# brownvc/matryodshka

Hardware: AMD Instinct MI355X
Metric: novel-view frames/sec, 640x320 ODS->32-sphere MSI infer+render (higher is better)
Workload: dtype f32

## Files before the change

matryodshka_amd/csrc/cnn_x3.hip:

```cpp
#include "cnn_device.h"

namespace {

#ifndef MSI_X3_EARLY_DMA
#define MSI_X3_EARLY_DMA 0
#endif
#ifndef MSI_X3_NSTG
#define MSI_X3_NSTG 0
#endif
#ifndef MSI_X2_NSTG
#define MSI_X2_NSTG 3
#endif
constexpr int x3_rate_y(int RATE) { return RATE == 3 ? 1 : RATE; }
constexpr int x3_rate_x(int RATE) { return RATE == 3 ? 2 : RATE; }
constexpr int x3_nstg(int RATE, int NPL) { return NPL == 2 ? MSI_X2_NSTG : (MSI_X3_NSTG ? MSI_X3_NSTG : (RATE == 2 ? 3 : 2)); }
template <int RATE, int NS = x3_nstg(RATE, 3), int NPL = 3, int TH = 4>
struct HaloGeomX3 {
  static constexpr int PW = 16 + 2 * x3_rate_x(RATE), PH = TH + 2 * x3_rate_y(RATE), NPX = PW * PH;
  static constexpr int PIX_BYTES = NPL * 64 + 16;
  static constexpr int ROW_PITCH = ((PW * PIX_BYTES + 127) / 256) * 256 + 128;
  static constexpr int A_BYTES = PH * ROW_PITCH;
  static constexpr int B_ROW = 64;
  static constexpr int B_PLANE = 64 * B_ROW, B_STAGE = NPL * B_PLANE;
  static constexpr int NSTG = NS;
// ... 42 lines not shown
    asm("v_cvt_pk_bf16_f32 %0, %1, %2" : "=v"(h1) : "v"(y.z), "v"(y.w));
    v4f r = y - v4f{__builtin_bit_cast(float, h0 << 16), __builtin_bit_cast(float, h0 & 0xffff0000u),
                    __builtin_bit_cast(float, h1 << 16), __builtin_bit_cast(float, h1 & 0xffff0000u)};
    asm("v_cvt_pk_bf16_f32 %0, %1, %2" : "=v"(m0) : "v"(r.x), "v"(r.y));
    asm("v_cvt_pk_bf16_f32 %0, %1, %2" : "=v"(m1) : "v"(r.z), "v"(r.w));
    r = r - v4f{__builtin_bit_cast(float, m0 << 16), __builtin_bit_cast(float, m0 & 0xffff0000u),
                __builtin_bit_cast(float, m1 << 16), __builtin_bit_cast(float, m1 & 0xffff0000u)};
    asm("v_cvt_pk_bf16_f32 %0, %1, %2" : "=v"(l0) : "v"(r.x), "v"(r.y));
    asm("v_cvt_pk_bf16_f32 %0, %1, %2" : "=v"(l1) : "v"(r.z), "v"(r.w));
    if (off != 0xffffffffu) {
      *reinterpret_cast<u2x_t *>(smem + off) = u2x_t{h0, h1};
      *reinterpret_cast<u2x_t *>(smem + off + 64) = u2x_t{m0, m1};
      *reinterpret_cast<u2x_t *>(smem + off + 128) = u2x_t{l0, l1};
    }
  }
}
template <int NP>
__device__ __forceinline__ void split_mfma(f32x16 &acc, f32x16 &lo, const v4f &ah, const v4f &am, const v4f &al, const v4f &bh, const v4f &bm, const v4f &bl) {
  typedef __bf16 bf16x8 __attribute__((ext_vector_type(8)));
  typedef _Float16 f16x8 __attribute__((ext_vector_type(8)));
  if (NP == 2) {
    lo = __builtin_amdgcn_mfma_f32_32x32x16_f16(__builtin_bit_cast(f16x8, bm), __builtin_bit_cast(f16x8, ah), lo, 0, 0, 0);
    acc = __builtin_amdgcn_mfma_f32_32x32x16_f16(__builtin_bit_cast(f16x8, bh), __builtin_bit_cast(f16x8, ah), acc, 0, 0, 0);
    lo = __builtin_amdgcn_mfma_f32_32x32x16_f16(__builtin_bit_cast(f16x8, bh), __builtin_bit_cast(f16x8, am), lo, 0, 0, 0);
  } else if (NP == 6) {
    acc = __builtin_amdgcn_mfma_f32_32x32x16_bf16(__builtin_bit_cast(bf16x8, bm), __builtin_bit_cast(bf16x8, am), acc, 0, 0, 0);
    acc = __builtin_amdgcn_mfma_f32_32x32x16_bf16(__builtin_bit_cast(bf16x8, bh), __builtin_bit_cast(bf16x8, al), acc, 0, 0, 0);
    acc = __builtin_amdgcn_mfma_f32_32x32x16_bf16(__builtin_bit_cast(bf16x8, bl), __builtin_bit_cast(bf16x8, ah), acc, 0, 0, 0);
    acc = __builtin_amdgcn_mfma_f32_32x32x16_bf16(__builtin_bit_cast(bf16x8, bh), __builtin_bit_cast(bf16x8, am), acc, 0, 0, 0);
    acc = __builtin_amdgcn_mfma_f32_32x32x16_bf16(__builtin_bit_cast(bf16x8, bm), __builtin_bit_cast(bf16x8, ah), acc, 0, 0, 0);
// ... 97 lines not shown
    }
  };
  auto patch_store = [&]() __attribute__((always_inline)) {
    v4f s4 = {1.f, 1.f, 1.f, 1.f}, t4 = {0.f, 0.f, 0.f, 0.f};
    if (APPLY) ln_scale_shift(ln, g4, be4, s4, t4);
#pragma unroll
    for (int k_ = 0; k_ < NLOAD; ++k_) {
      v4f y = araw[k_];
      if (APPLY) {
        y = __builtin_elementwise_max(__builtin_elementwise_fma(y, s4, t4), v4f{0.f, 0.f, 0.f, 0.f});
        if (has_pad && !pok[k_]) y = v4f{0.f, 0.f, 0.f, 0.f};
      }
      split_store<NPL>(smem, lds_a[k_], y, amax_);
    }
  };
  const int frow = lane & 31, fh = lane >> 5, fswz = (frow >> 1) & 7;
  const unsigned lds_base = (unsigned)(size_t)(lds_void *)smem;
  const unsigned a_base = lds_base + (unsigned)((2 * MT * wm + (frow >> 4)) * G::ROW_PITCH + ((frow & 15) ^ ((frow >> 4) << 3)) * G::PIX_BYTES + fh * 16);
  unsigned b_s[2];
  (void)fswz;
#pragma unroll
  for (int s_ = 0; s_ < 2; ++s_)
    b_s[s_] = lds_base + G::A_BYTES + (wn * 32 + frow) * G::B_ROW + (((2 * s_ + fh) ^ ((frow >> 2) & 3)) << 4);
  typedef _Float16 f16x8 __attribute__((ext_vector_type(8)));
  f32x16 acc[MT][1], acc_lo, acc_lo1;
#pragma unroll
  for (int i = 0; i < MT; ++i)
#pragma unroll
    for (int r = 0; r < 16; ++r) acc[i][0][r] = acc_lo[r] = acc_lo1[r] = 0.f;

// ... 58 lines not shown
    } else {
#pragma unroll
      for (int s_ = 0; s_ < 2; ++s_) {
      ah_[s_] = s_ == 0 ? lds_read128<AOFF_>(a_base) : lds_read128<AOFF_ + 32>(a_base);
      bh_[s_] = lds_read128<0>(b_s[s_] + bst_);
      am_[s_] = s_ == 0 ? lds_read128<AOFF_ + 64>(a_base) : lds_read128<AOFF_ + 96>(a_base);
      bm_[s_] = lds_read128<G::B_PLANE>(b_s[s_] + bst_);
      al_[s_] = s_ == 0 ? lds_read128<AOFF_ + 128>(a_base) : lds_read128<AOFF_ + 160>(a_base);
      bl_[s_] = lds_read128<2 * G::B_PLANE>(b_s[s_] + bst_);
    }
#pragma unroll
      for (int s_ = 0; s_ < 2; ++s_) {
      if (s_ == 0) wait_lgkm6<6>(ah_[0], bh_[0], am_[0], bm_[0], al_[0], bl_[0]);
      else wait_lgkm6<0>(ah_[1], bh_[1], am_[1], bm_[1], al_[1], bl_[1]);
      split_mfma<3>(acc[0][0], acc_lo, ah_[s_], am_[s_], al_[s_], bh_[s_], bm_[s_], bl_[s_]);
      __builtin_amdgcn_sched_barrier(0);
      if (s_ == 0) {
        if (TAP == 0 && c + 1 < c1) patch_load(c + 1);
        if (!MSI_X3_EARLY_DMA && G::NSTG == 3) {
        if (TAP + 2 < 9) { b_issue(c, TAP + 2, (TAP + 2) % 3); }
        else if (c + 1 < c1) { b_issue(c + 1, TAP - 7, (TAP + 2) % 3); }
        }
      }
    }
    }
    {
      const bool issued_ = (TAP + 2 < 9) || (c + 1 < c1);
      if (G::NSTG == 2) {
        if (TAP == 0 && c + 1 < c1) wait_vmcnt<NLOAD + (APPLY ? 2 : 0)>();
        else wait_vmcnt<0>();
// ... 9 lines not shown
    double *s_stat = reinterpret_cast<double *>(smem);
    ln_mean_inv_pre(shard, p.ln_inv_n, p.ln_scl_src, p.status, s_stat, tid);
    ln = ln_affine_read(s_stat);
  }
  wait_vmcnt<0>();
  patch_store();
  asm volatile("s_waitcnt lgkmcnt(0)" ::: "memory");
  __builtin_amdgcn_s_barrier();
#ifdef MSI_CONV_TIMING
  const unsigned long long ts1 = __builtin_amdgcn_s_memtime();
#endif
  for (; c < c1; ++c) {
    cpar = (c - c0) & 1;
    htap(IC<0>{}); htap(IC<1>{}); htap(IC<2>{}); htap(IC<3>{}); htap(IC<4>{}); htap(IC<5>{}); htap(IC<6>{}); htap(IC<7>{}); htap(IC<8>{});
    if (c + 1 < c1) {
      patch_store();
      asm volatile("s_waitcnt lgkmcnt(0)" ::: "memory");
      __builtin_amdgcn_s_barrier();
    }
  }
  if (MSI_X2_LATE_CB && NPL == 2) load_coord_bias(p, tile_m, tile_n, tid, cbv);
  split_finish<NPL>(acc[0][0], acc_lo, amax_, lane, p.status);
  if constexpr (MT == 2 && NPL == 3) split_finish<3>(acc[1][0], acc_lo1, amax_, lane, p.status);

#ifdef MSI_CONV_TIMING
  const unsigned long long ts2 = __builtin_amdgcn_s_memtime();
  auto stamp = [&]() __attribute__((always_inline)) {
    if (p.dbg && tid == 0) {
      unsigned long long *o = p.dbg + (size_t)blockIdx.x * 24;
      o[0] = ts0; o[1] = ts1; o[2] = ts2; o[3] = __builtin_amdgcn_s_memtime(); o[22] = ts0r; o[23] = __builtin_amdgcn_s_memrealtime();
      o[4] = __builtin_amdgcn_s_getreg(4 | (31 << 11));
// ... 61 lines not shown
  static constexpr int B_ROW = 64, B_PLANE = 64 * B_ROW, B_STAGE = NP * B_PLANE;
  static constexpr int NSTG = NP == 3 ? MSI_S2X3_NSTG : 3;
  static constexpr int LDS_BYTES = A_BYTES + NSTG * B_STAGE;
  static constexpr int NLOAD = (NPX * 8 + 255) / 256;
};

#ifndef MSI_S2X_WAVES
#define MSI_S2X_WAVES 3
#endif
template <int APPLY, int NP, int TH>
__device__ __forceinline__ void conv_halo_s2_x3_body(const ConvParams &p, char *smem) {
  typedef HaloGeomS2X3<NP, TH> G;
  constexpr int PW = G::PW, NPX = G::NPX, NLOAD = G::NLOAD;
  constexpr int MT = TH / 4, NT = 1, BM = 16 * TH;
  static_assert(TH == 4 || (TH == 8 && NP == 3 && G::NSTG == 2), "the 8-row tile: six-product form, two-stage ring");
  const int tid = threadIdx.x, lane = tid & 63;
  const int wave = __builtin_amdgcn_readfirstlane(tid >> 6);
  const int wm = wave >> 1, wn = wave & 1;
  const int CH = p.cpt0;
  const TileWork w = tile_work(p, CH);
  const int c0 = w.k0, c1 = w.k1;
  const TileIndex ti = tile_index(p, w.t);
  const int tile_m = ti.tile_m, tile_n = ti.tile_n, b = ti.b;
  const int tyi = (int)udiv_magic((unsigned)tile_m, (unsigned)p.halo_tx, p.mg_htx);
  const int oh0 = tyi * TH, ow0 = (tile_m - tyi * p.halo_tx) * 16;
  const int H = p.Hin, W = p.Win, C = p.C0;
  const int S = p.ksteps;
  const int plane_bytes = p.npad * G::B_ROW;
  const __amdgpu_buffer_rsrc_t rsrc_b = __builtin_amdgcn_make_buffer_rsrc((void *)p.wpk_x3, 0, (int)((size_t)S * NP * plane_bytes), 0x00020000);
  const unsigned b_voff = (unsigned)((tile_n * 64 + wave * 16 + (lane >> 2)) * G::B_ROW + (lane & 3) * 16);
// ... 61 lines not shown
    }
  };
  auto patch_store = [&](auto U_c) __attribute__((always_inline)) {
    constexpr int U = decltype(U_c)::value;
    if (APPLY && U == 0) ln_scale_shift(LnAffine{inv_f, mu_hi, mu_lo}, g4, be4, s4, t4);
#pragma unroll
    for (int k_ = 0; k_ < NLOAD; ++k_) {
      v4f y = araw[k_];
      if (APPLY) {
        y = __builtin_elementwise_max(__builtin_elementwise_fma(y, s4, t4), v4f{0.f, 0.f, 0.f, 0.f});
        if (has_pad && !pok[U][k_]) y = v4f{0.f, 0.f, 0.f, 0.f};
      }
      split_store<NP>(smem, lds_a[k_], y, amax_);
    }
  };

  const int frow = lane & 31, fh = lane >> 5, fswz = (frow >> 1) & 7;
  const unsigned lds_base = (unsigned)(size_t)(lds_void *)smem;
  const unsigned a_base = lds_base + (unsigned)((2 * MT * wm + (frow >> 4)) * G::ROW_PITCH + ((frow & 15) ^ ((frow >> 4) << 3)) * G::PIX_BYTES + fh * 16);
  unsigned b_s[2];
  (void)fswz;
#pragma unroll
  for (int s_ = 0; s_ < 2; ++s_)
    b_s[s_] = lds_base + G::A_BYTES + (wn * 32 + frow) * G::B_ROW + (((2 * s_ + fh) ^ ((frow >> 2) & 3)) << 4);
  typedef __bf16 bf16x8 __attribute__((ext_vector_type(8), unused));
  f32x16 acc[MT][1], acc_lo, acc_lo1;
#pragma unroll
  for (int r = 0; r < 16; ++r) {
    acc_lo[r] = acc_lo1[r] = 0.f;
#pragma unroll
// ... 12 lines not shown
    if (G::NSTG == 2) {
      const int stn_ = ((J ^ cpar) & 1) ^ 1;
      if (J + 1 < 9) b_issue(c, s2_tap((J + 1) % 9), stn_);
      else if (c + 1 < c1) b_issue(c + 1, s2_tap(0), stn_);
    }
    v4f ah_[2], am_[2], al_[2], bh_[2], bm_[2], bl_[2];
    if constexpr (MT == 2) {
      constexpr int A1_ = AOFF_ + 2 * G::ROW_PITCH;
      v4f xh_[2][2], xm_[2][2], xl_[2][2];
      bh_[0] = lds_read128<0>(b_s[0] + bst_); bm_[0] = lds_read128<G::B_PLANE>(b_s[0] + bst_); bl_[0] = lds_read128<2 * G::B_PLANE>(b_s[0] + bst_);
      xh_[0][0] = lds_read128<AOFF_>(a_base); xm_[0][0] = lds_read128<AOFF_ + 64>(a_base); xl_[0][0] = lds_read128<AOFF_ + 128>(a_base);
      xh_[0][1] = lds_read128<A1_>(a_base); xm_[0][1] = lds_read128<A1_ + 64>(a_base); xl_[0][1] = lds_read128<A1_ + 128>(a_base);
      bh_[1] = lds_read128<0>(b_s[1] + bst_); bm_[1] = lds_read128<G::B_PLANE>(b_s[1] + bst_); bl_[1] = lds_read128<2 * G::B_PLANE>(b_s[1] + bst_);
      wait_lgkm6<6>(bh_[0], bm_[0], bl_[0], xh_[0][0], xm_[0][0], xl_[0][0]);
      split_mfma<3>(acc[0][0], acc_lo, xh_[0][0], xm_[0][0], xl_[0][0], bh_[0], bm_[0], bl_[0]);
      __builtin_amdgcn_sched_barrier(0);
      xh_[1][0] = lds_read128<AOFF_ + 32>(a_base); xm_[1][0] = lds_read128<AOFF_ + 96>(a_base); xl_[1][0] = lds_read128<AOFF_ + 160>(a_base);
      xh_[1][1] = lds_read128<A1_ + 32>(a_base); xm_[1][1] = lds_read128<A1_ + 96>(a_base); xl_[1][1] = lds_read128<A1_ + 160>(a_base);
      if (FIRST_ && more_) {
        if (U_ < 3) patch_load(c, IC<(U_ + 1) & 3>{});
        else patch_load(c + 1, IC<0>{});
      }
      wait_lgkm6<9>(xh_[0][1], xm_[0][1], xl_[0][1], bh_[0], bm_[0], bl_[0]);
      split_mfma<3>(acc[1][0], acc_lo1, xh_[0][1], xm_[0][1], xl_[0][1], bh_[0], bm_[0], bl_[0]);
      __builtin_amdgcn_sched_barrier(0);
      wait_lgkm6<3>(bh_[1], bm_[1], bl_[1], xh_[1][0], xm_[1][0], xl_[1][0]);
      split_mfma<3>(acc[0][0], acc_lo, xh_[1][0], xm_[1][0], xl_[1][0], bh_[1], bm_[1], bl_[1]);
      __builtin_amdgcn_sched_barrier(0);
      wait_lgkm6<0>(xh_[1][1], xm_[1][1], xl_[1][1], bh_[1], bm_[1], bl_[1]);
      split_mfma<3>(acc[1][0], acc_lo1, xh_[1][1], xm_[1][1], xl_[1][1], bh_[1], bm_[1], bl_[1]);
      __builtin_amdgcn_sched_barrier(0);
    } else {
#pragma unroll
    for (int s_ = 0; s_ < 2; ++s_) {
      ah_[s_] = s_ == 0 ? lds_read128<AOFF_>(a_base) : lds_read128<AOFF_ + 32>(a_base);
      bh_[s_] = lds_read128<0>(b_s[s_] + bst_);
      am_[s_] = s_ == 0 ? lds_read128<AOFF_ + 64>(a_base) : lds_read128<AOFF_ + 96>(a_base);
      bm_[s_] = lds_read128<G::B_PLANE>(b_s[s_] + bst_);
      if (NP == 3) {
        al_[s_] = s_ == 0 ? lds_read128<AOFF_ + 128>(a_base) : lds_read128<AOFF_ + 160>(a_base);
        bl_[s_] = lds_read128<2 * G::B_PLANE>(b_s[s_] + bst_);
      } else { al_[s_] = ah_[s_]; bl_[s_] = bh_[s_]; }
    }
#pragma unroll
    for (int s_ = 0; s_ < 2; ++s_) {
      if (NP == 3) {
        if (s_ == 0) wait_lgkm6<6>(ah_[0], bh_[0], am_[0], bm_[0], al_[0], bl_[0]);
        else wait_lgkm6<0>(ah_[1], bh_[1], am_[1], bm_[1], al_[1], bl_[1]);
      } else {
        if (s_ == 0) wait_lgkm4<4>(ah_[0], bh_[0], am_[0], bm_[0]);
        else wait_lgkm4<0>(ah_[1], bh_[1], am_[1], bm_[1]);
      }
      split_mfma<NP>(acc[0][0], acc_lo, ah_[s_], am_[s_], al_[s_], bh_[s_], bm_[s_], bl_[s_]);
      __builtin_amdgcn_sched_barrier(0);
      if (s_ == 0) {
        if (FIRST_ && more_) {
          if (U_ < 3) patch_load(c, IC<(U_ + 1) & 3>{});
          else patch_load(c + 1, IC<0>{});
        }
        if (G::NSTG == 3) {
        if (J + 2 < 9) b_issue(c, s2_tap((J + 2) % 9), (J + 2) % 3);
        else if (c + 1 < c1) b_issue(c + 1, s2_tap((J + 2) % 9), (J + 2) % 3);
        }
      }
    }
    }
    {
      const bool issued_ = (J + 2 < 9) || (c + 1 < c1);
      if (G::NSTG == 2) {
        if (FIRST_ && !LAST_ && more_) wait_vmcnt<NLOAD>();
        else wait_vmcnt<0>();
      } else if (FIRST_ && !LAST_ && more_) wait_vmcnt<NP + NLOAD>();
      else if (issued_) wait_vmcnt<NP>();
      else wait_vmcnt<0>();
    }
    __builtin_amdgcn_s_barrier();
    if (LAST_ && more_) {
      patch_store(IC<(U_ + 1) & 3>{});
      asm volatile("s_waitcnt lgkmcnt(0)" ::: "memory");
      __builtin_amdgcn_s_barrier();
    }
  };

  if (APPLY) {
    double *s_stat = reinterpret_cast<double *>(smem);
    ln_mean_inv(p.ln_sums + (size_t)b * LN_SHARDS * LN_WORDS, p.ln_inv_n, p.ln_scl_src, p.status, s_stat, tid);
    const LnAffine a = ln_affine_read(s_stat);
    inv_f = a.inv; mu_hi = a.mu_hi; mu_lo = a.mu_lo;
  }
  wait_vmcnt<0>();
  patch_store(IC<0>{});
  asm volatile("s_waitcnt lgkmcnt(0)" ::: "memory");
  __builtin_amdgcn_s_barrier();
  for (; c < c1; ++c) {
    cpar = (c - c0) & 1;
    s2step(IC<0>{}); s2step(IC<1>{}); s2step(IC<2>{}); s2step(IC<3>{}); s2step(IC<4>{});
    s2step(IC<5>{}); s2step(IC<6>{}); s2step(IC<7>{}); s2step(IC<8>{});
  }
  split_finish<NP>(acc[0][0], acc_lo, amax_, lane, p.status);
  if constexpr (MT == 2 && NP == 3) split_finish<3>(acc[1][0], acc_lo1, amax_, lane, p.status);

  if (!w.full) {
    if (!splitk_arrive<MT, NT>(p, acc, w, smem, tid)) return;
    splitk_sum<MT, NT>(p, acc, w, tid);
  }
  emit_tile<BM, 64, MODE_CONV>(p, acc, tile_m, tile_n, 0, b, tid, smem);
}

template <int APPLY, int NP>
__global__ void __launch_bounds__(256) __attribute__((amdgpu_waves_per_eu(NP == 2 ? MSI_S2X_WAVES : (MSI_S2X3_NSTG == 2 ? 3 : 2))))
conv_halo_s2_x3_kernel(const ConvParams p) {
#if defined(__HIP_DEVICE_COMPILE__)
  extern __shared__ __attribute__((aligned(16))) char smem[];
  conv_halo_s2_x3_body<APPLY, NP, 4>(p, smem);
#endif
}

template <int APPLY>
__global__ void __launch_bounds__(256) __attribute__((amdgpu_waves_per_eu(2)))
conv_halo8_s2_x3_kernel(const ConvParams p) {
#if defined(__HIP_DEVICE_COMPILE__)
// ... 11 lines not shown
  static constexpr int NLOAD = (NPX * 8 + 255) / 256;
};
#ifndef MSI_CT_MAXW
#define MSI_CT_MAXW 8
#endif
#ifndef MSI_CT3_NSTG
#define MSI_CT3_NSTG 2
#endif
template <int NP, int TH>
__device__ __forceinline__ void convt_halo_x3_body(const ConvParams &p, char *smem) {
  typedef HaloGeomCT3<(NP == 3 ? MSI_CT3_NSTG : 3), NP, TH> G;
  constexpr int PW = G::PW, NPX = G::NPX, NLOAD = G::NLOAD, NSTG = G::NSTG, PD = NSTG - 1;
  constexpr int MT = TH / 4, BM = 16 * TH;
  static_assert(NSTG == 3 || NSTG == 2, "prefetch distance two or one");
  static_assert(TH == 4 || (TH == 8 && NP == 3 && NSTG == 2), "the 8-row tile: six-product form, two-stage ring");
  const int tid = threadIdx.x, lane = tid & 63;
  const int wave = __builtin_amdgcn_readfirstlane(tid >> 6);
  const int wm = wave >> 1, wn = wave & 1;
  const int CH = p.cpt0 + p.cpt1;
  const TileWork w = tile_work(p, CH);
  const int c0 = w.k0, c1 = w.k1;
  const TileIndex ti = tile_index<TILE_ROW_PARITY>(p, w.t);
  const int ph = ti.cls, tile_m = ti.tile_m, tile_n = ti.tile_n, b = ti.b;
  const int tyi = (int)udiv_magic((unsigned)tile_m, (unsigned)p.halo_tx, p.mg_htx);
  const int oh0 = tyi * TH, ow0 = (tile_m - tyi * p.halo_tx) * 16;
  const int H = p.Hin, W = p.Win;
  const int rowup = (ph && !p.wrap) ? 0 : 1;

  const int S = p.ksteps;
  const int plane_bytes = p.npad * G::B_ROW;
// ... 74 lines not shown
      const float ih_ = src_ld ? inv_f[1] : inv_f[0], mh_ = src_ld ? mu_hi[1] : mu_hi[0], ml_ = src_ld ? mu_lo[1] : mu_lo[0];
      s4 = ih_ * g4;
      const v4f nh = {-mh_, -mh_, -mh_, -mh_}, nl = {-ml_, -ml_, -ml_, -ml_};
      t4 = __builtin_elementwise_fma(nl, s4, __builtin_elementwise_fma(nh, s4, be4));
    }
#pragma unroll
    for (int k_ = 0; k_ < NLOAD; ++k_) {
      v4f y = araw[k_];
      if (ap_) {
        y = __builtin_elementwise_max(__builtin_elementwise_fma(y, s4, t4), v4f{0.f, 0.f, 0.f, 0.f});
        if (has_pad && !pok[k_]) y = v4f{0.f, 0.f, 0.f, 0.f};
      }
      split_store<NP>(smem, lds_a[k_], y, amax_);
    }
  };

  const int frow = lane & 31, fh = lane >> 5, fswz = (frow >> 1) & 7;
  const unsigned lds_base = (unsigned)(size_t)(lds_void *)smem;
  const unsigned a_base0 = lds_base + (unsigned)((rowup + 2 * MT * wm + (frow >> 4)) * G::ROW_PITCH + ((frow & 15) ^ ((frow >> 4) << 3)) * G::PIX_BYTES + fh * 16);
  const unsigned a_base1 = rowup ? a_base0 - G::ROW_PITCH : a_base0 + G::ROW_PITCH;
  const unsigned wadj = p.wrap ? 2u * G::PIX_BYTES : 0u;
  unsigned b_s[2];
  (void)fswz;
#pragma unroll
  for (int s_ = 0; s_ < 2; ++s_)
    b_s[s_] = lds_base + G::A_BYTES + (wn * 32 + frow) * G::B_ROW + (((2 * s_ + fh) ^ ((frow >> 2) & 3)) << 4);
  typedef __bf16 bf16x8 __attribute__((ext_vector_type(8), unused));
  f32x16 acc[2][MT][1], acc_lo[2];
#pragma unroll
  for (int cl = 0; cl < 2; ++cl)
#pragma unroll
    for (int r = 0; r < 16; ++r) {
      acc_lo[cl][r] = 0.f;
#pragma unroll
      for (int i = 0; i < MT; ++i) acc[cl][i][0][r] = 0.f;
    }

  int c = c0, st = 0;
  constexpr int NPLD = NLOAD + 2;
  auto ctstep = [&](auto J_c) __attribute__((always_inline)) {
    constexpr int J = decltype(J_c)::value;
    constexpr int PWC_ = J >> 2, TH_ = (J >> 1) & 1, TW_ = J & 1;
    constexpr int COFF_ = (1 + (PWC_ ? TW_ : -TW_)) * G::PIX_BYTES;
    const unsigned ab_ = (TH_ ? a_base1 : a_base0) - ((PWC_ && TW_) ? wadj : 0u);
    v4f ah_[2], am_[2], al_[2], bh_[2], bm_[2], bl_[2];
    const unsigned bst_ = (unsigned)st * G::B_STAGE;
    bool issued_ = false;
    if (NSTG == 2) {
      constexpr int JN_ = (J + 1) & 7;
      if (J + 1 < 8) { issued_ = true; b_issue(2 * ph + (JN_ >> 2), JN_ & 3, c, st ^ 1); }
      else if (c + 1 < c1) { issued_ = true; b_issue(2 * ph + (JN_ >> 2), JN_ & 3, c + 1, st ^ 1); }
    }
    if constexpr (MT == 2) {
      constexpr int C1_ = COFF_ + 2 * G::ROW_PITCH;
      v4f xh_[2][2], xm_[2][2], xl_[2][2];
      bh_[0] = lds_read128<0>(b_s[0] + bst_); bm_[0] = lds_read128<G::B_PLANE>(b_s[0] + bst_); bl_[0] = lds_read128<2 * G::B_PLANE>(b_s[0] + bst_);
      xh_[0][0] = lds_read128<COFF_>(ab_); xm_[0][0] = lds_read128<COFF_ + 64>(ab_); xl_[0][0] = lds_read128<COFF_ + 128>(ab_);
      xh_[0][1] = lds_read128<C1_>(ab_); xm_[0][1] = lds_read128<C1_ + 64>(ab_); xl_[0][1] = lds_read128<C1_ + 128>(ab_);
      bh_[1] = lds_read128<0>(b_s[1] + bst_); bm_[1] = lds_read128<G::B_PLANE>(b_s[1] + bst_); bl_[1] = lds_read128<2 * G::B_PLANE>(b_s[1] + bst_);
      wait_lgkm6<6>(bh_[0], bm_[0], bl_[0], xh_[0][0], xm_[0][0], xl_[0][0]);
      split_mfma<6>(acc[PWC_][0][0], acc_lo[PWC_], xh_[0][0], xm_[0][0], xl_[0][0], bh_[0], bm_[0], bl_[0]);
      __builtin_amdgcn_sched_barrier(0);
      xh_[1][0] = lds_read128<COFF_ + 32>(ab_); xm_[1][0] = lds_read128<COFF_ + 96>(ab_); xl_[1][0] = lds_read128<COFF_ + 160>(ab_);
      xh_[1][1] = lds_read128<C1_ + 32>(ab_); xm_[1][1] = lds_read128<C1_ + 96>(ab_); xl_[1][1] = lds_read128<C1_ + 160>(ab_);
      if (J == 0 && c + 1 < c1) patch_load(c + 1);
      wait_lgkm6<9>(xh_[0][1], xm_[0][1], xl_[0][1], bh_[0], bm_[0], bl_[0]);
      split_mfma<6>(acc[PWC_][1][0], acc_lo[PWC_], xh_[0][1], xm_[0][1], xl_[0][1], bh_[0], bm_[0], bl_[0]);
      __builtin_amdgcn_sched_barrier(0);
      wait_lgkm6<3>(bh_[1], bm_[1], bl_[1], xh_[1][0], xm_[1][0], xl_[1][0]);
      split_mfma<6>(acc[PWC_][0][0], acc_lo[PWC_], xh_[1][0], xm_[1][0], xl_[1][0], bh_[1], bm_[1], bl_[1]);
      __builtin_amdgcn_sched_barrier(0);
      wait_lgkm6<0>(xh_[1][1], xm_[1][1], xl_[1][1], bh_[1], bm_[1], bl_[1]);
      split_mfma<6>(acc[PWC_][1][0], acc_lo[PWC_], xh_[1][1], xm_[1][1], xl_[1][1], bh_[1], bm_[1], bl_[1]);
      __builtin_amdgcn_sched_barrier(0);
    } else {
#pragma unroll
    for (int s_ = 0; s_ < 2; ++s_) {
      ah_[s_] = s_ == 0 ? lds_read128<COFF_>(ab_) : lds_read128<COFF_ + 32>(ab_);
      bh_[s_] = lds_read128<0>(b_s[s_] + bst_);
      am_[s_] = s_ == 0 ? lds_read128<COFF_ + 64>(ab_) : lds_read128<COFF_ + 96>(ab_);
      bm_[s_] = lds_read128<G::B_PLANE>(b_s[s_] + bst_);
      if (NP == 3) {
        al_[s_] = s_ == 0 ? lds_read128<COFF_ + 128>(ab_) : lds_read128<COFF_ + 160>(ab_);
        bl_[s_] = lds_read128<2 * G::B_PLANE>(b_s[s_] + bst_);
      } else { al_[s_] = ah_[s_]; bl_[s_] = bh_[s_]; }
    }
#pragma unroll
    for (int s_ = 0; s_ < 2; ++s_) {
      if (NP == 3) {
        if (s_ == 0) wait_lgkm6<6>(ah_[0], bh_[0], am_[0], bm_[0], al_[0], bl_[0]);
        else wait_lgkm6<0>(ah_[1], bh_[1], am_[1], bm_[1], al_[1], bl_[1]);
      } else {
        if (s_ == 0) wait_lgkm4<4>(ah_[0], bh_[0], am_[0], bm_[0]);
        else wait_lgkm4<0>(ah_[1], bh_[1], am_[1], bm_[1]);
      }
      split_mfma<NP>(acc[PWC_][0][0], acc_lo[PWC_], ah_[s_], am_[s_], al_[s_], bh_[s_], bm_[s_], bl_[s_]);
      __builtin_amdgcn_sched_barrier(0);
      if (s_ == 0) {
        if (J == 0 && c + 1 < c1) patch_load(c + 1);
        if (NSTG == 3) {
        int sn_ = st + PD; sn_ = sn_ >= NSTG ? sn_ - NSTG : sn_;
        constexpr int JN_ = (J + PD) & 7;
        if (J + PD < 8) { issued_ = true; b_issue(2 * ph + (JN_ >> 2), JN_ & 3, c, sn_); }
        else if (c + 1 < c1) { issued_ = true; b_issue(2 * ph + (JN_ >> 2), JN_ & 3, c + 1, sn_); }
        }
      }
    }
    }
    if (NSTG == 2) {
      if (J == 0 && c + 1 < c1) wait_vmcnt<NPLD>();
      else wait_vmcnt<0>();
// ... 10 lines not shown
    if (p.halo_apply & 1) {
      ln_mean_inv(p.ln_sums + (size_t)b * LN_SHARDS * LN_WORDS, p.ln_inv_n, p.ln_scl_src, p.status, s_stat, tid);
      const LnAffine a = ln_affine_read(s_stat);
      inv_f[0] = a.inv; mu_hi[0] = a.mu_hi; mu_lo[0] = a.mu_lo;
    }
    if (p.halo_apply & 2) {
      ln_mean_inv(p.ln_sums1 + (size_t)b * LN_SHARDS * LN_WORDS, p.ln_inv_n1, p.ln_scl_src1, p.status, s_stat, tid);
      const LnAffine a = ln_affine_read(s_stat);
      inv_f[1] = a.inv; mu_hi[1] = a.mu_hi; mu_lo[1] = a.mu_lo;
    }
  }
  wait_vmcnt<0>();
  patch_store();
  asm volatile("s_waitcnt lgkmcnt(0)" ::: "memory");
  __builtin_amdgcn_s_barrier();
  for (; c < c1; ++c) {
    ctstep(IC<0>{}); ctstep(IC<1>{}); ctstep(IC<2>{}); ctstep(IC<3>{}); ctstep(IC<4>{}); ctstep(IC<5>{}); ctstep(IC<6>{}); ctstep(IC<7>{});
    if (c + 1 < c1) {
      patch_store();
      asm volatile("s_waitcnt lgkmcnt(0)" ::: "memory");
      __builtin_amdgcn_s_barrier();
    }
  }
  if constexpr (MT == 1) {
    split_finish<NP>(acc[0][0][0], acc_lo[0], amax_, lane, p.status);
    split_finish<NP>(acc[1][0][0], acc_lo[1], amax_, lane, p.status);
  }

  if (!w.full) {
    constexpr int SLAB = BM * 64 * 4;
    if (p.tile_cnt == nullptr) {
#pragma unroll
      for (int cl = 0; cl < 2; ++cl) {
        const __amdgpu_buffer_rsrc_t rsrc_p = __builtin_amdgcn_make_buffer_rsrc((void *)(p.partial + ((size_t)w.slot * 2 + cl) * (BM * 64)), 0, SLAB, 0x00020000);
        dump_acc<MT, 1, 0>(acc[cl], rsrc_p, tid);
      }
      return;
    }
#pragma unroll
    for (int cl = 0; cl < 2; ++cl) {
      const __amdgpu_buffer_rsrc_t rsrc_p = __builtin_amdgcn_make_buffer_rsrc((void *)(p.partial + ((size_t)w.slot * 2 + cl) * (BM * 64)), 0, SLAB, 0x00020000);
      dump_acc<MT, 1, MSI_HANDOFF_AUX>(acc[cl], rsrc_p, tid);
    }
    const int nsp = w.t < p.n_main ? p.split0 : p.split;
    asm volatile("s_waitcnt vmcnt(0)" ::: "memory");
    handoff_release();
    __syncthreads();
    int *s_old = reinterpret_cast<int *>(smem);
    if (tid == 0)
      *s_old = __hip_atomic_fetch_add(p.tile_cnt + (w.t - (p.split0 == 1 ? p.n_main : 0)), 1, __ATOMIC_RELAXED, __HIP_MEMORY_SCOPE_AGENT);
    __syncthreads();
    if (*s_old != nsp - 1) return;
    handoff_acquire();
#pragma unroll
    for (int cl = 0; cl < 2; ++cl) {
      const __amdgpu_buffer_rsrc_t rsrc_t = __builtin_amdgcn_make_buffer_rsrc((void *)(p.partial + ((size_t)(w.slot - w.ks) * 2 + cl) * (BM * 64)), 0, nsp * 2 * SLAB, 0x00020000);
      sum_slabs<MT, 1, MSI_HANDOFF_AUX>(acc[cl], rsrc_t, nsp, 2 * SLAB, tid);
    }
  }
#pragma unroll
  for (int cl = 0; cl < 2; ++cl) emit_tile<BM, 64, MODE_CONVT>(p, acc[cl], tile_m, tile_n, 2 * ph + cl, b, tid);
}

template <int NP>
__global__ void __launch_bounds__(256) __attribute__((amdgpu_waves_per_eu(NP == 3 ? 3 : 2, MSI_CT_MAXW)))
convt_halo_x3_kernel(const ConvParams p) {
#if defined(__HIP_DEVICE_COMPILE__)
  extern __shared__ __attribute__((aligned(16))) char smem[];
  convt_halo_x3_body<NP, 4>(p, smem);
#endif
}

__global__ void __launch_bounds__(256) __attribute__((amdgpu_waves_per_eu(2)))
convt_halo8_x3_kernel(const ConvParams p) {
#if defined(__HIP_DEVICE_COMPILE__)
  extern __shared__ __attribute__((aligned(16))) char smem[];
// ... 49 lines not shown
```

Before: 542.5.

## Interleave next-patch bf16 split with MFMA k-steps instead of at barrier

Moves the LayerNorm-affine, ReLU and three-plane bf16 split of the prefetched next input patch out of the serial store phase at each channel boundary. The work is spread into slots behind MFMA groups across the tap/k-step loop, using sched_group_barrier hints to interleave VALU with MFMA. The split planes are kept in registers and only written to LDS at the boundary. This adds register pressure (the extra plane arrays) and can perturb the schedule. The diff also adds optional timing instrumentation behind a macro.

```diff
diff --git a/matryodshka_amd/csrc/cnn_x3.hip b/matryodshka_amd/csrc/cnn_x3.hip
--- a/matryodshka_amd/csrc/cnn_x3.hip
+++ b/matryodshka_amd/csrc/cnn_x3.hip
@@ -2,6 +2,9 @@
 
 namespace {
 
+#ifndef MSI_EARLY_SPLIT
+#define MSI_EARLY_SPLIT 28
+#endif
 #ifndef MSI_X3_EARLY_DMA
 #define MSI_X3_EARLY_DMA 0
 #endif
@@ -80,6 +83,56 @@
       *reinterpret_cast<u2x_t *>(smem + off + 128) = u2x_t{l0, l1};
     }
   }
+}
+template <int NP>
+__device__ __forceinline__ void split_planes(v4f y, unsigned &amax, unsigned (&q)[2 * NP]) {
+  if constexpr (NP == 2) {
+    typedef _Float16 h2_t __attribute__((ext_vector_type(2)));
+    f16_range_track(amax, y);
+    const h2_t ha = {(_Float16)y.x, (_Float16)y.y}, hb = {(_Float16)y.z, (_Float16)y.w};
+    const h2_t ma = {(_Float16)((y.x - (float)ha.x) * 2048.f), (_Float16)((y.y - (float)ha.y) * 2048.f)};
+    const h2_t mb = {(_Float16)((y.z - (float)hb.x) * 2048.f), (_Float16)((y.w - (float)hb.y) * 2048.f)};
+    q[0] = __builtin_bit_cast(unsigned, ha); q[1] = __builtin_bit_cast(unsigned, hb);
+    q[2] = __builtin_bit_cast(unsigned, ma); q[3] = __builtin_bit_cast(unsigned, mb);
+  } else {
+    unsigned h0, h1, m0, m1, l0, l1;
+    asm("v_cvt_pk_bf16_f32 %0, %1, %2" : "=v"(h0) : "v"(y.x), "v"(y.y));
+    asm("v_cvt_pk_bf16_f32 %0, %1, %2" : "=v"(h1) : "v"(y.z), "v"(y.w));
+    v4f r = y - v4f{__builtin_bit_cast(float, h0 << 16), __builtin_bit_cast(float, h0 & 0xffff0000u),
+                    __builtin_bit_cast(float, h1 << 16), __builtin_bit_cast(float, h1 & 0xffff0000u)};
+    asm("v_cvt_pk_bf16_f32 %0, %1, %2" : "=v"(m0) : "v"(r.x), "v"(r.y));
+    asm("v_cvt_pk_bf16_f32 %0, %1, %2" : "=v"(m1) : "v"(r.z), "v"(r.w));
+    r = r - v4f{__builtin_bit_cast(float, m0 << 16), __builtin_bit_cast(float, m0 & 0xffff0000u),
+                __builtin_bit_cast(float, m1 << 16), __builtin_bit_cast(float, m1 & 0xffff0000u)};
+    asm("v_cvt_pk_bf16_f32 %0, %1, %2" : "=v"(l0) : "v"(r.x), "v"(r.y));
+    asm("v_cvt_pk_bf16_f32 %0, %1, %2" : "=v"(l1) : "v"(r.z), "v"(r.w));
+    q[0] = h0; q[1] = h1; q[2] = m0; q[3] = m1; q[4] = l0; q[5] = l1;
+  }
+}
+template <int NP>
+__device__ __forceinline__ void planes_store(char *smem, unsigned off, const unsigned (&q)[2 * NP]) {
+  typedef unsigned u2x_t __attribute__((ext_vector_type(2)));
+  if (off != 0xffffffffu) {
+    *reinterpret_cast<u2x_t *>(smem + off) = u2x_t{q[0], q[1]};
+    *reinterpret_cast<u2x_t *>(smem + off + 64) = u2x_t{q[2], q[3]};
+    if constexpr (NP == 3) *reinterpret_cast<u2x_t *>(smem + off + 128) = u2x_t{q[4], q[5]};
+  }
+}
+__device__ __forceinline__ void planes_keep(v4f &a, unsigned (&l)[2], const unsigned (&q)[6]) {
+  a = __builtin_bit_cast(v4f, u32x4_t{q[0], q[1], q[2], q[3]});
+  l[0] = q[4]; l[1] = q[5];
+}
+__device__ __forceinline__ void mfma_valu_interleave() {
+#pragma unroll
+  for (int i = 0; i < 6; ++i) {
+    __builtin_amdgcn_sched_group_barrier(0x008, 1, 0);
+    __builtin_amdgcn_sched_group_barrier(0x002, 7, 0);
+  }
+}
+__device__ __forceinline__ void planes_kept_store(char *smem, unsigned off, const v4f &a, const unsigned (&l)[2]) {
+  const u32x4_t hm = __builtin_bit_cast(u32x4_t, a);
+  const unsigned q[6] = {hm.x, hm.y, hm.z, hm.w, l[0], l[1]};
+  planes_store<3>(smem, off, q);
 }
 template <int NP>
 __device__ __forceinline__ void split_mfma(f32x16 &acc, f32x16 &lo, const v4f &ah, const v4f &am, const v4f &al, const v4f &bh, const v4f &bm, const v4f &bl) {
@@ -207,6 +260,35 @@
       split_store<NPL>(smem, lds_a[k_], y, amax_);
     }
   };
+  constexpr bool EARLY = TH == 4 && NPL == 3 && RATE != 2 && ((MSI_EARLY_SPLIT >> 4) & 1);
+  unsigned apl[EARLY ? NLOAD : 1][2];
+  auto early_slot = [&](auto TAP_c, auto Q_c) __attribute__((always_inline)) {
+    constexpr int k_ = decltype(Q_c)::value == 1 ? decltype(TAP_c)::value - (9 - NLOAD) : -1;
+    static_assert(NLOAD <= 7, "a slot per float4 of the patch, none before tap 2");
+    if constexpr (EARLY && k_ >= 0 && k_ < NLOAD) {
+      if (APPLY && k_ == 0) {
+        v4f s4 = {1.f, 1.f, 1.f, 1.f}, t4 = {0.f, 0.f, 0.f, 0.f};
+        ln_scale_shift(ln, g4, be4, s4, t4);
+        g4 = s4; be4 = t4;
+      }
+      v4f y = araw[k_];
+      if (APPLY) {
+        y = __builtin_elementwise_max(__builtin_elementwise_fma(y, g4, be4), v4f{0.f, 0.f, 0.f, 0.f});
+        const bool zero_ = has_pad && !pok[k_];
+        y.x = zero_ ? 0.f : y.x; y.y = zero_ ? 0.f : y.y; y.z = zero_ ? 0.f : y.z; y.w = zero_ ? 0.f : y.w;
+      }
+      unsigned q_[6];
+      split_planes<3>(y, amax_, q_);
+      planes_keep(araw[k_], apl[k_], q_);
+      mfma_valu_interleave();
+    }
+  };
+  auto early_store = [&]() __attribute__((always_inline)) {
+    if constexpr (EARLY) {
+#pragma unroll
+      for (int k_ = 0; k_ < NLOAD; ++k_) planes_kept_store(smem, lds_a[k_], araw[k_], apl[k_]);
+    }
+  };
   const int frow = lane & 31, fh = lane >> 5, fswz = (frow >> 1) & 7;
   const unsigned lds_base = (unsigned)(size_t)(lds_void *)smem;
   const unsigned a_base = lds_base + (unsigned)((2 * MT * wm + (frow >> 4)) * G::ROW_PITCH + ((frow & 15) ^ ((frow >> 4) << 3)) * G::PIX_BYTES + fh * 16);
@@ -295,6 +377,7 @@
       if (s_ == 0) wait_lgkm6<6>(ah_[0], bh_[0], am_[0], bm_[0], al_[0], bl_[0]);
       else wait_lgkm6<0>(ah_[1], bh_[1], am_[1], bm_[1], al_[1], bl_[1]);
       split_mfma<3>(acc[0][0], acc_lo, ah_[s_], am_[s_], al_[s_], bh_[s_], bm_[s_], bl_[s_]);
+      if (s_ == 0) early_slot(TAP_c, IC<0>{}); else early_slot(TAP_c, IC<1>{});
       __builtin_amdgcn_sched_barrier(0);
       if (s_ == 0) {
         if (TAP == 0 && c + 1 < c1) patch_load(c + 1);
@@ -334,7 +417,8 @@
     cpar = (c - c0) & 1;
     htap(IC<0>{}); htap(IC<1>{}); htap(IC<2>{}); htap(IC<3>{}); htap(IC<4>{}); htap(IC<5>{}); htap(IC<6>{}); htap(IC<7>{}); htap(IC<8>{});
     if (c + 1 < c1) {
-      patch_store();
+      if constexpr (EARLY) early_store();
+      else patch_store();
       asm volatile("s_waitcnt lgkmcnt(0)" ::: "memory");
       __builtin_amdgcn_s_barrier();
     }
@@ -426,6 +510,9 @@
   constexpr int PW = G::PW, NPX = G::NPX, NLOAD = G::NLOAD;
   constexpr int MT = TH / 4, NT = 1, BM = 16 * TH;
   static_assert(TH == 4 || (TH == 8 && NP == 3 && G::NSTG == 2), "the 8-row tile: six-product form, two-stage ring");
+#ifdef MSI_CONV_TIMING
+  const unsigned long long ts0 = __builtin_amdgcn_s_memtime(), ts0r = __builtin_amdgcn_s_memrealtime();
+#endif
   const int tid = threadIdx.x, lane = tid & 63;
   const int wave = __builtin_amdgcn_readfirstlane(tid >> 6);
   const int wm = wave >> 1, wn = wave & 1;
@@ -517,6 +604,42 @@
       split_store<NP>(smem, lds_a[k_], y, amax_);
     }
   };
+  constexpr bool EARLY = NP == 3 && ((MSI_EARLY_SPLIT >> (TH == 8 ? 3 : 2)) & 1);
+  unsigned apl[EARLY ? NLOAD : 1][2];
+  auto early_split = [&](auto U_c, auto K_c) __attribute__((always_inline)) {
+    constexpr int U = decltype(U_c)::value, k_ = decltype(K_c)::value;
+    if constexpr (EARLY && k_ >= 0 && k_ < NLOAD) {
+      v4f y = araw[k_];
+      if (APPLY) {
+        y = __builtin_elementwise_max(__builtin_elementwise_fma(y, s4, t4), v4f{0.f, 0.f, 0.f, 0.f});
+        const bool zero_ = has_pad && !pok[U][k_];
+        y.x = zero_ ? 0.f : y.x; y.y = zero_ ? 0.f : y.y; y.z = zero_ ? 0.f : y.z; y.w = zero_ ? 0.f : y.w;
+      }
+      unsigned q_[6];
+      split_planes<3>(y, amax_, q_);
+      planes_keep(araw[k_], apl[k_], q_);
+    }
+  };
+  auto early_slot = [&](auto J_c, auto Q_c) __attribute__((always_inline)) {
+    constexpr int J = decltype(J_c)::value, U_ = s2_unit(J), NG_ = 2 * MT, Q_ = decltype(Q_c)::value;
+    constexpr int E_ = U_ == 0 ? 2 : (U_ == 3 ? 0 : 1), LASTJ_ = U_ == 0 ? 3 : (U_ == 1 ? 5 : (U_ == 2 ? 7 : 8));
+    constexpr int NS_ = E_ * NG_, SLOT_ = Q_ < 0 ? -1 : (J - (LASTJ_ - E_ + 1)) * NG_ + Q_;
+    constexpr int SPS_ = NS_ ? (NLOAD + NS_ - 1) / NS_ : 0, K0_ = NLOAD - (NS_ - SLOT_) * SPS_;
+    static_assert(SPS_ <= 3, "at most three float4s behind one MFMA group");
+    if constexpr (EARLY && E_ > 0 && SLOT_ >= 0) {
+      if constexpr (SLOT_ == 0 && E_ == 1) wait_vmcnt<NP>();
+      early_split(IC<(U_ + 1) & 3>{}, IC<K0_>{});
+      if constexpr (SPS_ >= 2) early_split(IC<(U_ + 1) & 3>{}, IC<K0_ + 1>{});
+      if constexpr (SPS_ == 3) early_split(IC<(U_ + 1) & 3>{}, IC<K0_ + 2>{});
+      if constexpr (K0_ + SPS_ > 0) mfma_valu_interleave();
+    }
+  };
+  auto early_store = [&]() __attribute__((always_inline)) {
+    if constexpr (EARLY) {
+#pragma unroll
+      for (int k_ = 0; k_ < NLOAD; ++k_) planes_kept_store(smem, lds_a[k_], araw[k_], apl[k_]);
+    }
+  };
 
   const int frow = lane & 31, fh = lane >> 5, fswz = (frow >> 1) & 7;
   const unsigned lds_base = (unsigned)(size_t)(lds_void *)smem;
@@ -559,6 +682,7 @@
       bh_[1] = lds_read128<0>(b_s[1] + bst_); bm_[1] = lds_read128<G::B_PLANE>(b_s[1] + bst_); bl_[1] = lds_read128<2 * G::B_PLANE>(b_s[1] + bst_);
       wait_lgkm6<6>(bh_[0], bm_[0], bl_[0], xh_[0][0], xm_[0][0], xl_[0][0]);
       split_mfma<3>(acc[0][0], acc_lo, xh_[0][0], xm_[0][0], xl_[0][0], bh_[0], bm_[0], bl_[0]);
+      early_slot(J_c, IC<0>{});
       __builtin_amdgcn_sched_barrier(0);
       xh_[1][0] = lds_read128<AOFF_ + 32>(a_base); xm_[1][0] = lds_read128<AOFF_ + 96>(a_base); xl_[1][0] = lds_read128<AOFF_ + 160>(a_base);
       xh_[1][1] = lds_read128<A1_ + 32>(a_base); xm_[1][1] = lds_read128<A1_ + 96>(a_base); xl_[1][1] = lds_read128<A1_ + 160>(a_base);
@@ -568,12 +692,15 @@
       }
       wait_lgkm6<9>(xh_[0][1], xm_[0][1], xl_[0][1], bh_[0], bm_[0], bl_[0]);
       split_mfma<3>(acc[1][0], acc_lo1, xh_[0][1], xm_[0][1], xl_[0][1], bh_[0], bm_[0], bl_[0]);
+      early_slot(J_c, IC<1>{});
       __builtin_amdgcn_sched_barrier(0);
       wait_lgkm6<3>(bh_[1], bm_[1], bl_[1], xh_[1][0], xm_[1][0], xl_[1][0]);
       split_mfma<3>(acc[0][0], acc_lo, xh_[1][0], xm_[1][0], xl_[1][0], bh_[1], bm_[1], bl_[1]);
+      early_slot(J_c, IC<2>{});
       __builtin_amdgcn_sched_barrier(0);
       wait_lgkm6<0>(xh_[1][1], xm_[1][1], xl_[1][1], bh_[1], bm_[1], bl_[1]);
       split_mfma<3>(acc[1][0], acc_lo1, xh_[1][1], xm_[1][1], xl_[1][1], bh_[1], bm_[1], bl_[1]);
+      early_slot(J_c, IC<3>{});
       __builtin_amdgcn_sched_barrier(0);
     } else {
 #pragma unroll
@@ -597,6 +724,7 @@
         else wait_lgkm4<0>(ah_[1], bh_[1], am_[1], bm_[1]);
       }
       split_mfma<NP>(acc[0][0], acc_lo, ah_[s_], am_[s_], al_[s_], bh_[s_], bm_[s_], bl_[s_]);
+      if (s_ == 0) early_slot(J_c, IC<0>{}); else early_slot(J_c, IC<1>{});
       __builtin_amdgcn_sched_barrier(0);
       if (s_ == 0) {
         if (FIRST_ && more_) {
@@ -621,7 +749,8 @@
     }
     __builtin_amdgcn_s_barrier();
     if (LAST_ && more_) {
-      patch_store(IC<(U_ + 1) & 3>{});
+      if constexpr (EARLY && U_ < 3) early_store();
+      else patch_store(IC<(U_ + 1) & 3>{});
       asm volatile("s_waitcnt lgkmcnt(0)" ::: "memory");
       __builtin_amdgcn_s_barrier();
     }
@@ -637,6 +766,9 @@
   patch_store(IC<0>{});
   asm volatile("s_waitcnt lgkmcnt(0)" ::: "memory");
   __builtin_amdgcn_s_barrier();
+#ifdef MSI_CONV_TIMING
+  const unsigned long long ts1 = __builtin_amdgcn_s_memtime();
+#endif
   for (; c < c1; ++c) {
     cpar = (c - c0) & 1;
     s2step(IC<0>{}); s2step(IC<1>{}); s2step(IC<2>{}); s2step(IC<3>{}); s2step(IC<4>{});
@@ -645,11 +777,32 @@
   split_finish<NP>(acc[0][0], acc_lo, amax_, lane, p.status);
   if constexpr (MT == 2 && NP == 3) split_finish<3>(acc[1][0], acc_lo1, amax_, lane, p.status);
 
+#ifdef MSI_CONV_TIMING
+  const unsigned long long ts2 = __builtin_amdgcn_s_memtime();
+  auto stamp = [&]() __attribute__((always_inline)) {
+    if (p.dbg && threadIdx.x == 0) {
+      unsigned long long *o = p.dbg + (size_t)blockIdx.x * 24;
+      o[0] = ts0; o[1] = ts1; o[2] = ts2; o[3] = __builtin_amdgcn_s_memtime(); o[22] = ts0r; o[23] = __builtin_amdgcn_s_memrealtime();
+      o[4] = __builtin_amdgcn_s_getreg(4 | (31 << 11));
+      o[5] = __builtin_amdgcn_s_getreg(20 | (31 << 11));
+    }
+  };
+#endif
   if (!w.full) {
+#ifdef MSI_CONV_TIMING
+    if (!splitk_arrive<MT, NT>(p, acc, w, smem, tid)) {
+      if (p.tile_cnt == nullptr) stamp();
+      return;
+    }
+#else
     if (!splitk_arrive<MT, NT>(p, acc, w, smem, tid)) return;
+#endif
     splitk_sum<MT, NT>(p, acc, w, tid);
   }
   emit_tile<BM, 64, MODE_CONV>(p, acc, tile_m, tile_n, 0, b, tid, smem);
+#ifdef MSI_CONV_TIMING
+  stamp();
+#endif
 }
 
 template <int APPLY, int NP>
@@ -691,6 +844,9 @@
   constexpr int MT = TH / 4, BM = 16 * TH;
   static_assert(NSTG == 3 || NSTG == 2, "prefetch distance two or one");
   static_assert(TH == 4 || (TH == 8 && NP == 3 && NSTG == 2), "the 8-row tile: six-product form, two-stage ring");
+#ifdef MSI_CONV_TIMING
+  const unsigned long long ts0 = __builtin_amdgcn_s_memtime(), ts0r = __builtin_amdgcn_s_memrealtime();
+#endif
   const int tid = threadIdx.x, lane = tid & 63;
   const int wave = __builtin_amdgcn_readfirstlane(tid >> 6);
   const int wm = wave >> 1, wn = wave & 1;
@@ -795,6 +951,35 @@
       split_store<NP>(smem, lds_a[k_], y, amax_);
     }
   };
+  constexpr bool EARLY = NP == 3 && ((MSI_EARLY_SPLIT >> (TH == 8 ? 1 : 0)) & 1);
+  unsigned apl[EARLY ? NLOAD : 1][2];
+  auto early_affine = [&]() __attribute__((always_inline)) {
+    const float ih_ = src_ld ? inv_f[1] : inv_f[0], mh_ = src_ld ? mu_hi[1] : mu_hi[0], ml_ = src_ld ? mu_lo[1] : mu_lo[0];
+    const v4f s4 = ih_ * g4;
+    const v4f nh = {-mh_, -mh_, -mh_, -mh_}, nl = {-ml_, -ml_, -ml_, -ml_};
+    const v4f t4 = __builtin_elementwise_fma(nl, s4, __builtin_elementwise_fma(nh, s4, be4));
+    g4 = s4; be4 = t4;
+  };
+  auto early_split = [&](auto K_c) __attribute__((always_inline)) {
+    constexpr int k_ = decltype(K_c)::value;
+    if constexpr (EARLY && k_ < NLOAD) {
+      if (k_ == 0) early_affine();
+      const bool ap_ = (p.halo_apply >> src_ld) & 1, zero_ = has_pad && !pok[k_];
+      v4f y = araw[k_];
+      const v4f ya = __builtin_elementwise_max(__builtin_elementwise_fma(y, g4, be4), v4f{0.f, 0.f, 0.f, 0.f});
+      y.x = ap_ ? (zero_ ? 0.f : ya.x) : y.x; y.y = ap_ ? (zero_ ? 0.f : ya.y) : y.y;
+      y.z = ap_ ? (zero_ ? 0.f : ya.z) : y.z; y.w = ap_ ? (zero_ ? 0.f : ya.w) : y.w;
+      unsigned q_[6];
+      split_planes<3>(y, amax_, q_);
+      planes_keep(araw[k_], apl[k_], q_);
+    }
+  };
+  auto early_store = [&]() __attribute__((always_inline)) {
+    if constexpr (EARLY) {
+#pragma unroll
+      for (int k_ = 0; k_ < NLOAD; ++k_) planes_kept_store(smem, lds_a[k_], araw[k_], apl[k_]);
+    }
+  };
 
   const int frow = lane & 31, fh = lane >> 5, fswz = (frow >> 1) & 7;
   const unsigned lds_base = (unsigned)(size_t)(lds_void *)smem;
@@ -819,6 +1004,14 @@
 
   int c = c0, st = 0;
   constexpr int NPLD = NLOAD + 2;
+  auto early_slot = [&](auto J_c, auto Q_c) __attribute__((always_inline)) {
+    constexpr int SLOT_ = MT == 2 ? (decltype(J_c)::value - 6) * 4 + decltype(Q_c)::value : (decltype(Q_c)::value == 1 ? decltype(J_c)::value - (8 - NLOAD) : -1);
+    static_assert(NLOAD <= 6, "a slot per float4 of the patch, none before k-step 2");
+    if constexpr (EARLY && SLOT_ >= 0 && SLOT_ < NLOAD) {
+      early_split(IC<SLOT_>{});
+      mfma_valu_interleave();
+    }
+  };
   auto ctstep = [&](auto J_c) __attribute__((always_inline)) {
     constexpr int J = decltype(J_c)::value;
     constexpr int PWC_ = J >> 2, TH_ = (J >> 1) & 1, TW_ = J & 1;
@@ -841,18 +1034,22 @@
       bh_[1] = lds_read128<0>(b_s[1] + bst_); bm_[1] = lds_read128<G::B_PLANE>(b_s[1] + bst_); bl_[1] = lds_read128<2 * G::B_PLANE>(b_s[1] + bst_);
       wait_lgkm6<6>(bh_[0], bm_[0], bl_[0], xh_[0][0], xm_[0][0], xl_[0][0]);
       split_mfma<6>(acc[PWC_][0][0], acc_lo[PWC_], xh_[0][0], xm_[0][0], xl_[0][0], bh_[0], bm_[0], bl_[0]);
+      early_slot(J_c, IC<0>{});
       __builtin_amdgcn_sched_barrier(0);
       xh_[1][0] = lds_read128<COFF_ + 32>(ab_); xm_[1][0] = lds_read128<COFF_ + 96>(ab_); xl_[1][0] = lds_read128<COFF_ + 160>(ab_);
       xh_[1][1] = lds_read128<C1_ + 32>(ab_); xm_[1][1] = lds_read128<C1_ + 96>(ab_); xl_[1][1] = lds_read128<C1_ + 160>(ab_);
       if (J == 0 && c + 1 < c1) patch_load(c + 1);
       wait_lgkm6<9>(xh_[0][1], xm_[0][1], xl_[0][1], bh_[0], bm_[0], bl_[0]);
       split_mfma<6>(acc[PWC_][1][0], acc_lo[PWC_], xh_[0][1], xm_[0][1], xl_[0][1], bh_[0], bm_[0], bl_[0]);
+      early_slot(J_c, IC<1>{});
       __builtin_amdgcn_sched_barrier(0);
       wait_lgkm6<3>(bh_[1], bm_[1], bl_[1], xh_[1][0], xm_[1][0], xl_[1][0]);
       split_mfma<6>(acc[PWC_][0][0], acc_lo[PWC_], xh_[1][0], xm_[1][0], xl_[1][0], bh_[1], bm_[1], bl_[1]);
+      early_slot(J_c, IC<2>{});
       __builtin_amdgcn_sched_barrier(0);
       wait_lgkm6<0>(xh_[1][1], xm_[1][1], xl_[1][1], bh_[1], bm_[1], bl_[1]);
       split_mfma<6>(acc[PWC_][1][0], acc_lo[PWC_], xh_[1][1], xm_[1][1], xl_[1][1], bh_[1], bm_[1], bl_[1]);
+      early_slot(J_c, IC<3>{});
       __builtin_amdgcn_sched_barrier(0);
     } else {
 #pragma unroll
@@ -876,6 +1073,7 @@
         else wait_lgkm4<0>(ah_[1], bh_[1], am_[1], bm_[1]);
       }
       split_mfma<NP>(acc[PWC_][0][0], acc_lo[PWC_], ah_[s_], am_[s_], al_[s_], bh_[s_], bm_[s_], bl_[s_]);
+      if (s_ == 0) early_slot(J_c, IC<0>{}); else early_slot(J_c, IC<1>{});
       __builtin_amdgcn_sched_barrier(0);
       if (s_ == 0) {
         if (J == 0 && c + 1 < c1) patch_load(c + 1);
@@ -916,10 +1114,14 @@
   patch_store();
   asm volatile("s_waitcnt lgkmcnt(0)" ::: "memory");
   __builtin_amdgcn_s_barrier();
+#ifdef MSI_CONV_TIMING
+  const unsigned long long ts1 = __builtin_amdgcn_s_memtime();
+#endif
   for (; c < c1; ++c) {
     ctstep(IC<0>{}); ctstep(IC<1>{}); ctstep(IC<2>{}); ctstep(IC<3>{}); ctstep(IC<4>{}); ctstep(IC<5>{}); ctstep(IC<6>{}); ctstep(IC<7>{});
     if (c + 1 < c1) {
-      patch_store();
+      if constexpr (EARLY) early_store();
+      else patch_store();
       asm volatile("s_waitcnt lgkmcnt(0)" ::: "memory");
       __builtin_amdgcn_s_barrier();
     }
@@ -929,6 +1131,17 @@
     split_finish<NP>(acc[1][0][0], acc_lo[1], amax_, lane, p.status);
   }
 
+#ifdef MSI_CONV_TIMING
+  const unsigned long long ts2 = __builtin_amdgcn_s_memtime();
+  auto stamp = [&]() __attribute__((always_inline)) {
+    if (p.dbg && threadIdx.x == 0) {
+      unsigned long long *o = p.dbg + (size_t)blockIdx.x * 24;
+      o[0] = ts0; o[1] = ts1; o[2] = ts2; o[3] = __builtin_amdgcn_s_memtime(); o[22] = ts0r; o[23] = __builtin_amdgcn_s_memrealtime();
+      o[4] = __builtin_amdgcn_s_getreg(4 | (31 << 11));
+      o[5] = __builtin_amdgcn_s_getreg(20 | (31 << 11));
+    }
+  };
+#endif
   if (!w.full) {
     constexpr int SLAB = BM * 64 * 4;
     if (p.tile_cnt == nullptr) {
@@ -937,6 +1150,9 @@
         const __amdgpu_buffer_rsrc_t rsrc_p = __builtin_amdgcn_make_buffer_rsrc((void *)(p.partial + ((size_t)w.slot * 2 + cl) * (BM * 64)), 0, SLAB, 0x00020000);
         dump_acc<MT, 1, 0>(acc[cl], rsrc_p, tid);
       }
+#ifdef MSI_CONV_TIMING
+      stamp();
+#endif
       return;
     }
 #pragma unroll
@@ -962,6 +1178,9 @@
   }
 #pragma unroll
   for (int cl = 0; cl < 2; ++cl) emit_tile<BM, 64, MODE_CONVT>(p, acc[cl], tile_m, tile_n, 2 * ph + cl, b, tid);
+#ifdef MSI_CONV_TIMING
+  stamp();
+#endif
 }
 
 template <int NP>
```

After: 545.3, median of 6. About the same (+0.5%).
